# lim0606/pytorch-ardae-vae

Hardware: AMD Instinct MI355X
Metric: AR-DAE-VAE train-steps/sec (batch 512, nz_cdae 256) on dbMNIST (higher is better)
Workload: dtype f32; 1 GPU; BASELINE config #2: MNISTIPVAE mlp z=32 h=256 + cDAE mlp-grad h=256 L=3, global batch 512, nz_cdae 256 (131072 rows), dynamic binarisation on device, 1 cDAE + 1 VAE update per step; global_batch=512, nz_cdae=256, per_gpu_batch=512, parallelism=dp1

## Files before the change

pytorch-ardae-vae_amd/csrc/linear_narrow.hip:

```cpp
#include <stdlib.h>

#include "linear.h"
#include "profile.h"

namespace ardae {
namespace {

constexpr int NK = 32;

template <int EPI>
__global__ __launch_bounds__(256) void linear_narrow_kernel(const LinArgs a) {
  __shared__ float red[4];
  const int tid = threadIdx.x, lane = tid & 63, wave = tid >> 6;
  const int l31 = lane & 31, hh = lane >> 5;
  const int row0 = (blockIdx.x * 4 + wave) * 32;

  const float* xr = a.src[0].x + (size_t)(row0 + l31) * a.src[0].ld + 4 * hh;
  f32x4 av[NK];
#pragma unroll
  for (int c = 0; c < NK; ++c) av[c] = *reinterpret_cast<const f32x4*>(xr + 8 * c);

  const int col = min(l31, a.Nout - 1);
  const bool cok = l31 < a.Nout;
  const float bcol = a.bias ? a.bias[col] : 0.f;
  float sg[16], ev[16];
  if (EPI == EPI_DAE_LOSS) {
#pragma unroll
    for (int r = 0; r < 16; ++r) {
      const int row = row0 + (r & 3) + 8 * (r >> 2) + 4 * hh;
      sg[r] = a.sigma[row];
      ev[r] = a.eps[(size_t)row * a.ldeps + col];
    }
  }

  const float* bp = a.src[0].wp + lane * 4;
  f32x16 acc;
#pragma unroll
  for (int r = 0; r < 16; ++r) acc[r] = 0.f;
  f32x4 b0[8], b1[8];
#pragma unroll
  for (int u = 0; u < 8; ++u) b0[u] = *reinterpret_cast<const f32x4*>(bp + (size_t)u * 256);
#pragma unroll
  for (int g = 0; g < 4; g += 2) {
#pragma unroll
    for (int u = 0; u < 8; ++u) b1[u] = *reinterpret_cast<const f32x4*>(bp + (size_t)(8 * (g + 1) + u) * 256);
#pragma unroll
    for (int u = 0; u < 8; ++u)
#pragma unroll
      for (int q = 0; q < 4; ++q) acc = __builtin_amdgcn_mfma_f32_32x32x2f32(av[8 * g + u][q], b0[u][q], acc, 0, 0, 0);
    if (g + 2 < 4) {
#pragma unroll
      for (int u = 0; u < 8; ++u) b0[u] = *reinterpret_cast<const f32x4*>(bp + (size_t)(8 * (g + 2) + u) * 256);
    }
#pragma unroll
    for (int u = 0; u < 8; ++u)
#pragma unroll
      for (int q = 0; q < 4; ++q) acc = __builtin_amdgcn_mfma_f32_32x32x2f32(av[8 * (g + 1) + u][q], b1[u][q], acc, 0, 0, 0);
  }

  if (EPI == EPI_ACT) {
#pragma unroll
    for (int r = 0; r < 16; ++r) {
      const int row = row0 + (r & 3) + 8 * (r >> 2) + 4 * hh;
      if (cok) a.Y[(size_t)row * a.ldY + col] = acc[r] + bcol;
    }
  } else {
    float loss_part = 0.f;
#pragma unroll
    for (int r = 0; r < 16; ++r) {
      const int row = row0 + (r & 3) + 8 * (r >> 2) + 4 * hh;
      const float y = acc[r] + bcol;
      const float rho = sg[r] * y + ev[r];
      if (cok) {
        if (a.Y) a.Y[(size_t)row * a.ldY + col] = y;
        if (a.Y2) a.Y2[(size_t)row * a.ldY2 + col] = 2.f * sg[r] * rho * a.scale;
        loss_part += rho * rho;
      }
    }
#pragma unroll
    for (int off = 32; off > 0; off >>= 1) loss_part += __shfl_xor(loss_part, off);
    if (lane == 0) red[wave] = loss_part;
    __syncthreads();
    if (tid == 0) a.tile_loss[blockIdx.x] = (red[0] + red[1]) + (red[2] + red[3]);
  }
}

template <int EPI>
int launch_narrow(const LinArgs& a, hipStream_t st) {
  if (g_prof_enabled) {
    char name[64];
    snprintf(name, sizeof(name), "linear_narrow_kernel<%d>", EPI);
    const double tensors = EPI == EPI_DAE_LOSS ? (1.0 + (a.Y ? 1 : 0) + (a.Y2 ? 1 : 0)) : 1.0;
    prof_begin(st, name, 2.0 * a.M * (double)a.Nout * 256.0, 4.0 * ((double)a.M * 256.0 + tensors * a.M * (double)a.Nout + 256.0 * a.Nout));
  }
  hipLaunchKernelGGL((linear_narrow_kernel<EPI>), dim3(a.M / 128), dim3(256), 0, st, a);
  prof_end(st);
  ARDAE_LAUNCH_CHECK();
  return 0;
}

}

bool linear_narrow_eligible(const LinArgs& a, int epi) {
  static const bool on = !(debug_knob("ARDAE_NARROW") && atoi(debug_knob("ARDAE_NARROW")) == 0);
  if (!on || a.nsrc != 1 || a.src[0].K != 256 || a.Nout <= 0 || a.Nout > 32 || a.M <= 0 || (a.M % 128)) return false;
  if ((a.src[0].ld & 3) || (reinterpret_cast<uintptr_t>(a.src[0].x) & 15) || a.colsum != nullptr) return false;
  if (epi == EPI_ACT) return a.act == ACT_NONE && !a.rowbias && !a.rowscale && !a.Y2 && a.Y != nullptr;
  if (epi == EPI_DAE_LOSS) return a.tile_loss != nullptr && a.sigma != nullptr && a.eps != nullptr;
  return false;
}

int launch_linear_narrow(const LinArgs& a, int epi, hipStream_t st) {
  return epi == EPI_ACT ? launch_narrow<EPI_ACT>(a, st) : launch_narrow<EPI_DAE_LOSS>(a, st);
}

}
```

pytorch-ardae-vae_amd/csrc/wgrad_wide.hip:

```cpp
#include <stdlib.h>

#include "profile.h"
#include "wgrad.h"
#include "wgrad_wide_tiles.h"

namespace ardae {
namespace {

constexpr int WT = 256;
constexpr int WRC = 32;
constexpr int WCHUNK_BYTES = WRC * WT * 4;

template <int NA, int NB, int WOW>
struct WGeo {
  static constexpr int NA_ = NA, NB_ = NB;
  static constexpr int WIW = 4 / WOW;
  static constexpr int TO = NA * 32 * WOW, TI = NB * 32 * WIW;
  static constexpr int NM = NA * NB;
  static constexpr int XC4 = TI / 4;
  static constexpr int XRPP = 256 / XC4;
  static constexpr int NXP = WRC / XRPP;
  static constexpr int XCHUNK_BYTES = WRC * TI * 4;
  static constexpr int BUF_BYTES = WCHUNK_BYTES + XCHUNK_BYTES;
  static_assert(TO == WT, "the G staging layout assumes 256 output rows per tile");
};
using GeoSquare = WGeo<4, 4, 2>;
using GeoNarrow = WGeo<2, 1, 4>;

typedef __attribute__((address_space(3))) float lds_f32;



template <int OFF>
__device__ __forceinline__ void gload4(f32x4& dst, unsigned voff, const float* sbase) {
  asm volatile("s_nop 4\n\tglobal_load_dwordx4 %0, %1, %2 offset:%3" : "=v"(dst) : "v"(voff), "s"(sbase), "n"(OFF) : "memory");
}
template <int OFF>
__device__ __forceinline__ void gload1(float& dst, unsigned voff, const float* sbase) {
  asm volatile("s_nop 4\n\tglobal_load_dword %0, %1, %2 offset:%3" : "=v"(dst) : "v"(voff), "s"(sbase), "n"(OFF) : "memory");
}
template <int OFF>
__device__ __forceinline__ void lds_read1(float& dst, unsigned addr) {
  asm volatile("ds_read_b32 %0, %1 offset:%2" : "=v"(dst) : "v"(addr), "n"(OFF) : "memory");
}
template <int OFF>
__device__ __forceinline__ void lds_write4(unsigned addr, const f32x4& v) {
  asm volatile("ds_write_b128 %0, %1 offset:%2" ::"v"(addr), "v"(v), "n"(OFF) : "memory");
}

struct WwCtx {
  const float* gnext;
  const float* xnext;
  const float* rsnext;
  int ldg, ldx;
  unsigned gvoff, xvoff, rsvoff;
  unsigned gfrag, xfrag;
  unsigned gfrag_n, xfrag_n;
  unsigned gw, xw;
  float fb, fr;
};

template <class GEO>
struct Stage {
  static constexpr bool SQ = GEO::NM >= 8;
  static constexpr int PER = SQ ? 8 : 2;
  static constexpr int k_gl = 0, n_gl = 8 / PER;
  static constexpr int k_xl = k_gl + n_gl, n_xl = (GEO::NXP + PER - 1) / PER;
  static constexpr int k_rs = k_xl + n_xl, n_rs = 8 / PER;
  static constexpr int k_sum = 11;
  static constexpr int k_gw = 12, n_gw = SQ ? 1 : 2;
  static constexpr int k_xw = k_gw + n_gw;
  static_assert(k_rs + n_rs <= k_sum - 2 && k_xw <= 14, "stage schedule does not fit the chunk");
  static constexpr int count(int ks) {
    if (ks >= k_gl && ks < k_gl + n_gl) return PER;
    if (ks >= k_xl && ks < k_xl + n_xl) return (GEO::NXP - (ks - k_xl) * PER) < PER ? (GEO::NXP - (ks - k_xl) * PER) : PER;
    if (ks >= k_rs && ks < k_rs + n_rs) return PER;
    if (ks == k_sum) return 8;
    if (ks >= k_gw && ks < k_gw + n_gw) return 8 / n_gw;
    if (ks == k_xw) return GEO::NXP;
    return 0;
  }
};

template <class GEO, int KS, int J>
__device__ __forceinline__ void stage_op(f32x4 (&gv)[8], f32x4 (&xv)[GEO::NXP], float (&rs)[8], f32x4& bsum, f32x4& rsum, const WwCtx& c) {
  using ST = Stage<GEO>;
  if constexpr (KS >= ST::k_gl && KS < ST::k_gl + ST::n_gl) {
    constexpr int p = (KS - ST::k_gl) * ST::PER + J;
    gload4<0>(gv[p], c.gvoff, c.gnext + (size_t)(4 * p) * c.ldg);
  } else if constexpr (KS >= ST::k_xl && KS < ST::k_xl + ST::n_xl) {
    constexpr int p = (KS - ST::k_xl) * ST::PER + J;
    gload4<0>(xv[p], c.xvoff, c.xnext + (size_t)(GEO::XRPP * p) * c.ldx);
  } else if constexpr (KS >= ST::k_rs && KS < ST::k_rs + ST::n_rs) {
    constexpr int p = (KS - ST::k_rs) * ST::PER + J;
    gload1<16 * p>(rs[p], c.rsvoff, c.rsnext);
  } else if constexpr (KS == ST::k_sum) {
    if constexpr (J == 0) {
      asm volatile("s_waitcnt vmcnt(0)"
                   : "+v"(gv[0]), "+v"(gv[1]), "+v"(gv[2]), "+v"(gv[3]), "+v"(gv[4]), "+v"(gv[5]), "+v"(gv[6]), "+v"(gv[7])
                   :
                   : "memory");
      if constexpr (GEO::NXP == 8)
        asm volatile("s_waitcnt vmcnt(0)"
                     : "+v"(xv[0]), "+v"(xv[1]), "+v"(xv[2]), "+v"(xv[3]), "+v"(xv[4]), "+v"(xv[5]), "+v"(xv[6]), "+v"(xv[7])
                     :
                     : "memory");
      else asm volatile("s_waitcnt vmcnt(0)" : "+v"(xv[0]) : : "memory");
      asm volatile("s_waitcnt vmcnt(0)"
                   : "+v"(rs[0]), "+v"(rs[1]), "+v"(rs[2]), "+v"(rs[3]), "+v"(rs[4]), "+v"(rs[5]), "+v"(rs[6]), "+v"(rs[7])
                   :
                   : "memory");
    }
    bsum += gv[J] * c.fb;
    rsum += gv[J] * (rs[J] * c.fr);
  } else if constexpr (KS >= ST::k_gw && KS < ST::k_gw + ST::n_gw) {
    constexpr int p = (KS - ST::k_gw) * (8 / ST::n_gw) + J;
    lds_write4<p * 4096>(c.gw, gv[p]);
  } else if constexpr (KS == ST::k_xw) {
    lds_write4<J * GEO::XRPP * GEO::TI * 4>(c.xw, xv[J]);
  }
}

template <class GEO, int KS, int Q>
__device__ __forceinline__ void kstep_op(float (&A)[2][GEO::NA_], float (&B)[2][GEO::NB_], f32x4 (&gv)[8], f32x4 (&xv)[GEO::NXP], float (&rs)[8],
                                         f32x4& bsum, f32x4& rsum, const WwCtx& c) {
  constexpr int NA = GEO::NA_, NB = GEO::NB_;
  constexpr int nxt = (KS + 1) & 1;
  if constexpr (Q < NA) {
    if constexpr (KS < 15) lds_read1<(KS + 1) * 2048 + Q * 128>(A[nxt][Q], c.gfrag);
    else lds_read1<Q * 128>(A[nxt][Q], c.gfrag_n);
  } else if constexpr (Q < NA + NB) {
    constexpr int f = Q - NA;
    if constexpr (KS < 15) lds_read1<(KS + 1) * 2 * GEO::TI * 4 + f * 128>(B[nxt][f], c.xfrag);
    else lds_read1<f * 128>(B[nxt][f], c.xfrag_n);
  } else {
    stage_op<GEO, KS, Q - NA - NB>(gv, xv, rs, bsum, rsum, c);
  }
}

template <class GEO, int KS, int Q, int QEND>
__device__ __forceinline__ void kstep_ops(float (&A)[2][GEO::NA_], float (&B)[2][GEO::NB_], f32x4 (&gv)[8], f32x4 (&xv)[GEO::NXP], float (&rs)[8],
                                          f32x4& bsum, f32x4& rsum, const WwCtx& c) {
  if constexpr (Q < QEND) {
    kstep_op<GEO, KS, Q>(A, B, gv, xv, rs, bsum, rsum, c);
    kstep_ops<GEO, KS, Q + 1, QEND>(A, B, gv, xv, rs, bsum, rsum, c);
  }
}

template <class GEO, int KS, int S = 0>
__device__ __forceinline__ void kstep_mfmas(f32x16 (&acc)[GEO::NA_][GEO::NB_], float (&A)[2][GEO::NA_], float (&B)[2][GEO::NB_], f32x4 (&gv)[8],
                                            f32x4 (&xv)[GEO::NXP], float (&rs)[8], f32x4& bsum, f32x4& rsum, const WwCtx& c) {
  if constexpr (S < GEO::NM) {
    constexpr int a = S / GEO::NB_, b = S % GEO::NB_, cur = KS & 1;
    constexpr int total = GEO::NA_ + GEO::NB_ + Stage<GEO>::count(KS);
    constexpr int per = (total + GEO::NM - 1) / GEO::NM;
    constexpr int q0 = S * per < total ? S * per : total, q1 = (S + 1) * per < total ? (S + 1) * per : total;
    acc[a][b] = __builtin_amdgcn_mfma_f32_32x32x2f32(A[cur][a], B[cur][b], acc[a][b], 0, 0, 0);
    __builtin_amdgcn_sched_barrier(0);
    kstep_ops<GEO, KS, q0, q1>(A, B, gv, xv, rs, bsum, rsum, c);
    __builtin_amdgcn_sched_barrier(0);
    kstep_mfmas<GEO, KS, S + 1>(acc, A, B, gv, xv, rs, bsum, rsum, c);
  }
}

template <int N>
__device__ __forceinline__ void wait_frags(float (&v)[N]) {
  if constexpr (N == 4) asm volatile("s_waitcnt lgkmcnt(0)" : "+v"(v[0]), "+v"(v[1]), "+v"(v[2]), "+v"(v[3]) : : "memory");
  else if constexpr (N == 2) asm volatile("s_waitcnt lgkmcnt(0)" : "+v"(v[0]), "+v"(v[1]) : : "memory");
  else asm volatile("s_waitcnt lgkmcnt(0)" : "+v"(v[0]) : : "memory");
}

template <class GEO, int KS = 0>
__device__ __forceinline__ void chunk_ksteps(f32x16 (&acc)[GEO::NA_][GEO::NB_], float (&A)[2][GEO::NA_], float (&B)[2][GEO::NB_], f32x4 (&gv)[8],
                                             f32x4 (&xv)[GEO::NXP], float (&rs)[8], f32x4& bsum, f32x4& rsum, const WwCtx& c) {
  if constexpr (KS < 16) {
    constexpr int cur = KS & 1;
    wait_frags(A[cur]);
    wait_frags(B[cur]);
    if constexpr (KS == 15) __builtin_amdgcn_s_barrier();
    __builtin_amdgcn_sched_barrier(0);
    kstep_mfmas<GEO, KS>(acc, A, B, gv, xv, rs, bsum, rsum, c);
    chunk_ksteps<GEO, KS + 1>(acc, A, B, gv, xv, rs, bsum, rsum, c);
  }
}

template <class GEO>
__global__ __launch_bounds__(256, 1) void wgrad_wide_kernel(const WwBatchDev batch) {
  constexpr int NA = GEO::NA_, NB = GEO::NB_, NXP = GEO::NXP;
  __shared__ float lds[2 * GEO::BUF_BYTES / 4];
  const int tid = threadIdx.x, lane = tid & 63;
  const int wave = __builtin_amdgcn_readfirstlane(tid >> 6);
  const int l31 = lane & 31, hh = lane >> 5;
  const int wo = wave / GEO::WIW, wi = wave % GEO::WIW;
  const int ti = (int)blockIdx.x / batch.splits, split = (int)blockIdx.x - ti * batch.splits;
  const WwTile& T = batch.t[ti];

  const int cpp = T.M / WRC;
  const int ctot = cpp * T.npairs;
  const int cps = (ctot + batch.splits - 1) / batch.splits;
  const int c_begin = split * cps;
  const int c_end = c_begin + cps < ctot ? c_begin + cps : ctot;

  const unsigned lds0 = (unsigned)(uintptr_t)(lds_f32*)lds;
  const int sr = tid >> 6, sc4 = tid & 63;
  const int xr = tid / GEO::XC4, xc4 = tid % GEO::XC4;
  const unsigned gwbase = lds0 + (unsigned)((sr * WT + sc4 * 4) * 4);
  const unsigned xwbase = lds0 + WCHUNK_BYTES + (unsigned)((xr * GEO::TI + xc4 * 4) * 4);
  const unsigned gfrag0 = lds0 + (unsigned)((hh * WT + wo * NA * 32 + l31) * 4);
  const unsigned xfrag0 = lds0 + WCHUNK_BYTES + (unsigned)((hh * GEO::TI + wi * NB * 32 + l31) * 4);

  WwCtx c;
  auto chunk_ptrs = [&](int ch) {
    const int cc = ch < c_end ? ch : c_end - 1;
    const int pr = cc >= cpp ? 1 : 0;
    const int m0 = (cc - pr * cpp) * WRC;
    c.ldg = pr ? T.ldG[1] : T.ldG[0];
    c.ldx = pr ? T.ldX[1] : T.ldX[0];
    c.gnext = (pr ? T.G[1] : T.G[0]) + (size_t)m0 * c.ldg + T.o0;
    c.xnext = (pr ? T.X[1] : T.X[0]) + (size_t)m0 * c.ldx + T.i0;
    const bool vec = T.want_vec && pr == T.bias_pair && ch < c_end;
    c.fb = vec ? 1.f : 0.f;
    c.fr = (vec && T.rowscale) ? 1.f : 0.f;
    c.rsnext = T.rowscale ? T.rowscale + m0 : c.gnext;
    c.gvoff = (unsigned)((sr * c.ldg + sc4 * 4) * 4);
    c.xvoff = (unsigned)((xr * c.ldx + xc4 * 4) * 4);
    c.rsvoff = (unsigned)(sr * 4);
  };

  f32x16 acc[NA][NB];
#pragma unroll
  for (int a = 0; a < NA; ++a)
#pragma unroll
    for (int b = 0; b < NB; ++b)
#pragma unroll
      for (int r = 0; r < 16; ++r) acc[a][b][r] = 0.f;
  f32x4 bsum = {0.f, 0.f, 0.f, 0.f}, rsum = {0.f, 0.f, 0.f, 0.f};

  float A[2][NA], B[2][NB], rs[8];
  f32x4 gv[8], xv[NXP];
  if (c_begin < c_end) {
    chunk_ptrs(c_begin);
#pragma unroll
    for (int p = 0; p < 8; ++p) {
      gv[p] = *reinterpret_cast<const f32x4*>(c.gnext + (size_t)(4 * p + sr) * c.ldg + sc4 * 4);
      rs[p] = T.rowscale ? T.rowscale[(c.rsnext - T.rowscale) + 4 * p + sr] : 0.f;
    }
#pragma unroll
    for (int p = 0; p < NXP; ++p) xv[p] = *reinterpret_cast<const f32x4*>(c.xnext + (size_t)(GEO::XRPP * p + xr) * c.ldx + xc4 * 4);
#pragma unroll
    for (int p = 0; p < 8; ++p) {
      bsum += gv[p] * c.fb;
      rsum += gv[p] * (rs[p] * c.fr);
      *reinterpret_cast<f32x4*>(&lds[((4 * p + sr) * WT + sc4 * 4)]) = gv[p];
    }
#pragma unroll
    for (int p = 0; p < NXP; ++p) *reinterpret_cast<f32x4*>(&lds[WCHUNK_BYTES / 4 + (GEO::XRPP * p + xr) * GEO::TI + xc4 * 4]) = xv[p];
    __syncthreads();
#pragma unroll
    for (int f = 0; f < NA; ++f) A[0][f] = lds[hh * WT + wo * NA * 32 + f * 32 + l31];
#pragma unroll
    for (int f = 0; f < NB; ++f) B[0][f] = lds[WCHUNK_BYTES / 4 + hh * GEO::TI + wi * NB * 32 + f * 32 + l31];
    asm volatile("s_waitcnt vmcnt(0) lgkmcnt(0)" ::: "memory");

    int buf = 0;
    for (int ch = c_begin; ch < c_end; ++ch) {
      chunk_ptrs(ch + 1);
      const unsigned cur = (unsigned)buf * GEO::BUF_BYTES, oth = (unsigned)(buf ^ 1) * GEO::BUF_BYTES;
      c.gfrag = gfrag0 + cur; c.xfrag = xfrag0 + cur;
      c.gfrag_n = gfrag0 + oth; c.xfrag_n = xfrag0 + oth;
      c.gw = gwbase + oth; c.xw = xwbase + oth;
      chunk_ksteps<GEO, 0>(acc, A, B, gv, xv, rs, bsum, rsum, c);
      buf ^= 1;
    }
    wait_frags(A[0]);
    wait_frags(B[0]);
    asm volatile("s_waitcnt vmcnt(0) lgkmcnt(0)" ::: "memory");
  }

  float* __restrict__ part = T.partial + (size_t)split * T.O * T.I;
#pragma unroll
  for (int a = 0; a < NA; ++a) {
#pragma unroll
    for (int b = 0; b < NB; ++b) {
      const int i = T.i0 + wi * NB * 32 + b * 32 + l31;
#pragma unroll
      for (int r = 0; r < 16; ++r) {
        const int o = T.o0 + wo * NA * 32 + a * 32 + (r & 3) + 8 * (r >> 2) + 4 * hh;
        part[(size_t)o * T.I + i] = acc[a][b][r];
      }
    }
  }
  if (T.want_vec && T.i0 == 0) {
    __syncthreads();
    *reinterpret_cast<f32x4*>(&lds[sr * WT + sc4 * 4]) = bsum;
    *reinterpret_cast<f32x4*>(&lds[4 * WT + sr * WT + sc4 * 4]) = rsum;
    __syncthreads();
    const float s0 = (lds[tid] + lds[WT + tid]) + (lds[2 * WT + tid] + lds[3 * WT + tid]);
    const float s1 = (lds[4 * WT + tid] + lds[5 * WT + tid]) + (lds[6 * WT + tid] + lds[7 * WT + tid]);
    T.partial_vec[((size_t)split * 2 + 0) * T.O + T.o0 + tid] = s0;
    T.partial_vec[((size_t)split * 2 + 1) * T.O + T.o0 + tid] = s1;
  }
}

bool al16g(const void* p) { return (reinterpret_cast<uintptr_t>(p) & 15) == 0; }

}

int wgrad_wide_geometry(const WgradProblem& p) {
  static const bool off = debug_knob("ARDAE_WGRAD_WIDE") && atoi(debug_knob("ARDAE_WGRAD_WIDE")) == 0;
  if (off) return 0;
  if (p.O % WT || p.I % 32 || p.M % WRC || p.M < 64 * WRC) return 0;
  for (int k = 0; k < p.npairs; ++k) {
    if ((p.ldG[k] & 3) || (p.ldX[k] & 3) || !al16g(p.G[k]) || !al16g(p.X[k])) return 0;
    if ((int64_t)p.ldG[k] * 4 * 4 >= (int64_t)1 << 31 || (int64_t)p.ldX[k] * 32 * 4 >= (int64_t)1 << 31) return 0;
  }
  if (p.I % WT == 0) return 1;
  return p.I <= 64 ? 2 : 0;
}

bool wgrad_wide_eligible(const WgradProblem& p) { return wgrad_wide_geometry(p) != 0; }

template <class GEO>
int launch_wgrad_wide_geo(WgradProblem* probs, const int* idx, int n, hipStream_t st, const char* name) {
  if (n == 0) return 0;
  WwBatchDev b;
  memset(&b, 0, sizeof(b));
  int ntiles = 0, min_splits = 1 << 30;
  for (int k = 0; k < n; ++k) {
    const WgradProblem& p = probs[idx[k]];
    ntiles += (p.O / GEO::TO) * (p.I / GEO::TI);
    if (p.splits < min_splits) min_splits = p.splits;
  }
  ARDAE_CHECK_ARG(ntiles <= WW_MAX_TILES, "wgrad_wide: too many tiles (%d)", ntiles);
  int splits = 256 / ntiles;
  if (splits < 1) splits = 1;
  if (splits > min_splits) splits = min_splits;
  b.ntiles = ntiles;
  b.splits = splits;
  int t = 0;
  double fl = 0, by = 0;
  for (int k = 0; k < n; ++k) {
    WgradProblem& p = probs[idx[k]];
    p.splits = splits;
    for (int o0 = 0; o0 < p.O; o0 += GEO::TO)
      for (int i0 = 0; i0 < p.I; i0 += GEO::TI) {
        WwTile& w = b.t[t++];
        for (int q = 0; q < 2; ++q) {
          w.G[q] = p.G[q]; w.X[q] = p.X[q]; w.ldG[q] = p.ldG[q]; w.ldX[q] = p.ldX[q];
        }
        w.rowscale = p.rowscale; w.partial = p.partial; w.partial_vec = p.partial_vec;
        w.M = p.M; w.npairs = p.npairs; w.O = p.O; w.I = p.I; w.o0 = o0; w.i0 = i0;
        w.bias_pair = p.bias_pair; w.want_vec = (p.bias_pair >= 0 && p.partial_vec != nullptr) ? 1 : 0;
      }
    fl += 2.0 * p.npairs * (double)p.M * p.O * p.I;
    by += 4.0 * (p.npairs * (double)p.M * (p.O + p.I) + (double)splits * p.O * p.I);
  }
  bool x9 = GEO::TI == 256;
  for (int k = 0; x9 && k < n; ++k) x9 = wgrad_x9_eligible(probs[idx[k]]);
  if (g_prof_enabled) prof_begin(st, x9 ? "wgrad_x9_kernel<256x256>" : name, fl, by);
  if (x9) {
    ARDAE_TRY(launch_wgrad_x9(b, st));
  } else {
    hipLaunchKernelGGL(wgrad_wide_kernel<GEO>, dim3(ntiles * splits), dim3(256), 0, st, b);
  }
  prof_end(st);
  ARDAE_LAUNCH_CHECK();
  return n;
}

int launch_wgrad_wide(WgradProblem* probs, const int* idx, int n, hipStream_t st) {
  int sq[WGRAD_MAX_PROBLEMS], nr[WGRAD_MAX_PROBLEMS], nsq = 0, nnr = 0;
  for (int k = 0; k < n; ++k) {
    if (wgrad_wide_geometry(probs[idx[k]]) == 1) sq[nsq++] = idx[k];
    else nr[nnr++] = idx[k];
  }
  int rc = launch_wgrad_wide_geo<GeoSquare>(probs, sq, nsq, st, "wgrad_wide_kernel<256x256>");
  if (rc < 0) return rc;
  rc = launch_wgrad_wide_geo<GeoNarrow>(probs, nr, nnr, st, "wgrad_wide_kernel<256x32>");
  return rc < 0 ? rc : n;
}

}
```

Before: 223.8 train-steps/sec.

## Add persistent narrow-linear kernel and two-chunk-ahead prefetch in narrow wgrad

Adds a persistent version of the narrow (Nout<=32, K=256) linear kernel. It keeps the weight fragment in registers and double-buffers the next tile's activation rows while the current tile runs its MFMAs, which avoids reloading weights per tile and hides load latency. The narrow-geometry wgrad kernel now issues global loads two chunks ahead with two register sets and partial vmcnt waits, so fewer loads are exposed at each chunk boundary. The cost is higher register pressure, tricky waitcnt accounting and bias-vector bookkeeping, and a persistent grid hardcoded to 256 blocks.

```diff
diff --git a/pytorch-ardae-vae_amd/csrc/linear_narrow.hip b/pytorch-ardae-vae_amd/csrc/linear_narrow.hip
--- a/pytorch-ardae-vae_amd/csrc/linear_narrow.hip
+++ b/pytorch-ardae-vae_amd/csrc/linear_narrow.hip
@@ -85,6 +85,95 @@
   }
 }
 
+template <int EPI, int P>
+__device__ __forceinline__ void narrow_trip(const LinArgs& a, int t, int ntiles, f32x4 (&av)[2][NK], const f32x4 (&bw)[NK], float (&red)[2][4],
+                                            int tid, int lane, int wave, int col, bool cok, float bcol) {
+  const int l31 = lane & 31, hh = lane >> 5;
+  const int row0 = (t * 4 + wave) * 32;
+  float sg[16], ev[16];
+  if (EPI == EPI_DAE_LOSS) {
+#pragma unroll
+    for (int r = 0; r < 16; ++r) {
+      const int row = row0 + (r & 3) + 8 * (r >> 2) + 4 * hh;
+      sg[r] = a.sigma[row];
+      ev[r] = a.eps[(size_t)row * a.ldeps + col];
+    }
+  }
+  const int tn = t + (int)gridDim.x;
+  const float* xn = tn < ntiles ? a.src[0].x + (size_t)((tn * 4 + wave) * 32 + l31) * a.src[0].ld + 4 * hh : a.src[0].wp + 4 * hh;
+#pragma unroll
+  for (int c = 0; c < NK; ++c) av[P ^ 1][c] = *reinterpret_cast<const f32x4*>(xn + 8 * c);
+  __builtin_amdgcn_sched_barrier(0);
+
+  f32x16 acc;
+#pragma unroll
+  for (int r = 0; r < 16; ++r) acc[r] = 0.f;
+#pragma unroll
+  for (int c = 0; c < NK; ++c)
+#pragma unroll
+    for (int q = 0; q < 4; ++q) acc = __builtin_amdgcn_mfma_f32_32x32x2f32(av[P][c][q], bw[c][q], acc, 0, 0, 0);
+
+  if (EPI == EPI_ACT) {
+#pragma unroll
+    for (int r = 0; r < 16; ++r) {
+      const int row = row0 + (r & 3) + 8 * (r >> 2) + 4 * hh;
+      if (cok) a.Y[(size_t)row * a.ldY + col] = acc[r] + bcol;
+    }
+  } else {
+    float loss_part = 0.f;
+#pragma unroll
+    for (int r = 0; r < 16; ++r) {
+      const int row = row0 + (r & 3) + 8 * (r >> 2) + 4 * hh;
+      const float y = acc[r] + bcol;
+      const float rho = sg[r] * y + ev[r];
+      if (cok) {
+        if (a.Y) a.Y[(size_t)row * a.ldY + col] = y;
+        if (a.Y2) a.Y2[(size_t)row * a.ldY2 + col] = 2.f * sg[r] * rho * a.scale;
+        loss_part += rho * rho;
+      }
+    }
+#pragma unroll
+    for (int off = 32; off > 0; off >>= 1) loss_part += __shfl_xor(loss_part, off);
+    if (lane == 0) red[P][wave] = loss_part;
+    __syncthreads();
+    if (tid == 0) a.tile_loss[t] = (red[P][0] + red[P][1]) + (red[P][2] + red[P][3]);
+  }
+}
+
+template <int EPI>
+__global__ __launch_bounds__(256, 1) void linear_narrow_persistent_kernel(const LinArgs a, int ntiles) {
+  __shared__ float red[2][4];
+  const int tid = threadIdx.x, lane = tid & 63, wave = tid >> 6;
+  const int l31 = lane & 31, hh = lane >> 5;
+  int t = blockIdx.x;
+
+  f32x4 av[2][NK], bw[NK];
+  const float* xr = a.src[0].x + (size_t)((t * 4 + wave) * 32 + l31) * a.src[0].ld + 4 * hh;
+#pragma unroll
+  for (int c = 0; c < NK; ++c) av[0][c] = *reinterpret_cast<const f32x4*>(xr + 8 * c);
+  const float* bp = a.src[0].wp + lane * 4;
+#pragma unroll
+  for (int c = 0; c < NK; ++c) bw[c] = *reinterpret_cast<const f32x4*>(bp + (size_t)c * 256);
+  const int col = min(l31, a.Nout - 1);
+  const bool cok = l31 < a.Nout;
+  const float bcol = a.bias ? a.bias[col] : 0.f;
+
+  for (;;) {
+    narrow_trip<EPI, 0>(a, t, ntiles, av, bw, red, tid, lane, wave, col, cok, bcol);
+    t += (int)gridDim.x;
+    if (t >= ntiles) break;
+    narrow_trip<EPI, 1>(a, t, ntiles, av, bw, red, tid, lane, wave, col, cok, bcol);
+    t += (int)gridDim.x;
+    if (t >= ntiles) break;
+  }
+}
+
+constexpr int NARROW_CUS = 256;
+bool narrow_persistent(int ntiles) {
+  static const bool on = !(debug_knob("ARDAE_NARROW_PERSISTENT") && atoi(debug_knob("ARDAE_NARROW_PERSISTENT")) == 0);
+  return on && ntiles > 2 * NARROW_CUS;
+}
+
 template <int EPI>
 int launch_narrow(const LinArgs& a, hipStream_t st) {
   if (g_prof_enabled) {
@@ -93,7 +182,12 @@
     const double tensors = EPI == EPI_DAE_LOSS ? (1.0 + (a.Y ? 1 : 0) + (a.Y2 ? 1 : 0)) : 1.0;
     prof_begin(st, name, 2.0 * a.M * (double)a.Nout * 256.0, 4.0 * ((double)a.M * 256.0 + tensors * a.M * (double)a.Nout + 256.0 * a.Nout));
   }
-  hipLaunchKernelGGL((linear_narrow_kernel<EPI>), dim3(a.M / 128), dim3(256), 0, st, a);
+  const int ntiles = a.M / 128;
+  if (narrow_persistent(ntiles)) {
+    hipLaunchKernelGGL((linear_narrow_persistent_kernel<EPI>), dim3(NARROW_CUS), dim3(256), 0, st, a, ntiles);
+  } else {
+    hipLaunchKernelGGL((linear_narrow_kernel<EPI>), dim3(ntiles), dim3(256), 0, st, a);
+  }
   prof_end(st);
   ARDAE_LAUNCH_CHECK();
   return 0;
diff --git a/pytorch-ardae-vae_amd/csrc/wgrad_wide.hip b/pytorch-ardae-vae_amd/csrc/wgrad_wide.hip
--- a/pytorch-ardae-vae_amd/csrc/wgrad_wide.hip
+++ b/pytorch-ardae-vae_amd/csrc/wgrad_wide.hip
@@ -82,33 +82,42 @@
   }
 };
 
-template <class GEO, int KS, int J>
-__device__ __forceinline__ void stage_op(f32x4 (&gv)[8], f32x4 (&xv)[GEO::NXP], float (&rs)[8], f32x4& bsum, f32x4& rsum, const WwCtx& c) {
+template <class GEO, int AH, int LS, int KS, int J>
+__device__ __forceinline__ void stage_op(f32x4 (&gva)[AH][8], f32x4 (&xva)[AH][GEO::NXP], float (&rsa)[AH][8], f32x4& bsum, f32x4& rsum,
+                                         const WwCtx& c) {
   using ST = Stage<GEO>;
+  constexpr bool SAME = AH == 1 || LS == 2;
+  constexpr int L = LS & 1, CS = SAME ? L : L ^ 1, NEWER = SAME ? 0 : 8 + GEO::NXP + 8;
+  f32x4 (&gl)[8] = gva[L];
+  f32x4 (&xl)[GEO::NXP] = xva[L];
+  float (&rl)[8] = rsa[L];
+  f32x4 (&gv)[8] = gva[CS];
+  f32x4 (&xv)[GEO::NXP] = xva[CS];
+  float (&rs)[8] = rsa[CS];
   if constexpr (KS >= ST::k_gl && KS < ST::k_gl + ST::n_gl) {
     constexpr int p = (KS - ST::k_gl) * ST::PER + J;
-    gload4<0>(gv[p], c.gvoff, c.gnext + (size_t)(4 * p) * c.ldg);
+    gload4<0>(gl[p], c.gvoff, c.gnext + (size_t)(4 * p) * c.ldg);
   } else if constexpr (KS >= ST::k_xl && KS < ST::k_xl + ST::n_xl) {
     constexpr int p = (KS - ST::k_xl) * ST::PER + J;
-    gload4<0>(xv[p], c.xvoff, c.xnext + (size_t)(GEO::XRPP * p) * c.ldx);
+    gload4<0>(xl[p], c.xvoff, c.xnext + (size_t)(GEO::XRPP * p) * c.ldx);
   } else if constexpr (KS >= ST::k_rs && KS < ST::k_rs + ST::n_rs) {
     constexpr int p = (KS - ST::k_rs) * ST::PER + J;
-    gload1<16 * p>(rs[p], c.rsvoff, c.rsnext);
+    gload1<16 * p>(rl[p], c.rsvoff, c.rsnext);
   } else if constexpr (KS == ST::k_sum) {
     if constexpr (J == 0) {
-      asm volatile("s_waitcnt vmcnt(0)"
+      asm volatile("s_waitcnt vmcnt(%[n])"
                    : "+v"(gv[0]), "+v"(gv[1]), "+v"(gv[2]), "+v"(gv[3]), "+v"(gv[4]), "+v"(gv[5]), "+v"(gv[6]), "+v"(gv[7])
-                   :
+                   : [n] "n"(NEWER)
                    : "memory");
       if constexpr (GEO::NXP == 8)
-        asm volatile("s_waitcnt vmcnt(0)"
+        asm volatile("s_waitcnt vmcnt(%[n])"
                      : "+v"(xv[0]), "+v"(xv[1]), "+v"(xv[2]), "+v"(xv[3]), "+v"(xv[4]), "+v"(xv[5]), "+v"(xv[6]), "+v"(xv[7])
-                     :
+                     : [n] "n"(NEWER)
                      : "memory");
-      else asm volatile("s_waitcnt vmcnt(0)" : "+v"(xv[0]) : : "memory");
-      asm volatile("s_waitcnt vmcnt(0)"
+      else asm volatile("s_waitcnt vmcnt(%[n])" : "+v"(xv[0]) : [n] "n"(NEWER) : "memory");
+      asm volatile("s_waitcnt vmcnt(%[n])"
                    : "+v"(rs[0]), "+v"(rs[1]), "+v"(rs[2]), "+v"(rs[3]), "+v"(rs[4]), "+v"(rs[5]), "+v"(rs[6]), "+v"(rs[7])
-                   :
+                   : [n] "n"(NEWER)
                    : "memory");
     }
     bsum += gv[J] * c.fb;
@@ -121,9 +130,9 @@
   }
 }
 
-template <class GEO, int KS, int Q>
-__device__ __forceinline__ void kstep_op(float (&A)[2][GEO::NA_], float (&B)[2][GEO::NB_], f32x4 (&gv)[8], f32x4 (&xv)[GEO::NXP], float (&rs)[8],
-                                         f32x4& bsum, f32x4& rsum, const WwCtx& c) {
+template <class GEO, int AH, int LS, int KS, int Q>
+__device__ __forceinline__ void kstep_op(float (&A)[2][GEO::NA_], float (&B)[2][GEO::NB_], f32x4 (&gv)[AH][8], f32x4 (&xv)[AH][GEO::NXP],
+                                         float (&rs)[AH][8], f32x4& bsum, f32x4& rsum, const WwCtx& c) {
   constexpr int NA = GEO::NA_, NB = GEO::NB_;
   constexpr int nxt = (KS + 1) & 1;
   if constexpr (Q < NA) {
@@ -134,22 +143,22 @@
     if constexpr (KS < 15) lds_read1<(KS + 1) * 2 * GEO::TI * 4 + f * 128>(B[nxt][f], c.xfrag);
     else lds_read1<f * 128>(B[nxt][f], c.xfrag_n);
   } else {
-    stage_op<GEO, KS, Q - NA - NB>(gv, xv, rs, bsum, rsum, c);
-  }
-}
-
-template <class GEO, int KS, int Q, int QEND>
-__device__ __forceinline__ void kstep_ops(float (&A)[2][GEO::NA_], float (&B)[2][GEO::NB_], f32x4 (&gv)[8], f32x4 (&xv)[GEO::NXP], float (&rs)[8],
-                                          f32x4& bsum, f32x4& rsum, const WwCtx& c) {
+    stage_op<GEO, AH, LS, KS, Q - NA - NB>(gv, xv, rs, bsum, rsum, c);
+  }
+}
+
+template <class GEO, int AH, int LS, int KS, int Q, int QEND>
+__device__ __forceinline__ void kstep_ops(float (&A)[2][GEO::NA_], float (&B)[2][GEO::NB_], f32x4 (&gv)[AH][8], f32x4 (&xv)[AH][GEO::NXP],
+                                          float (&rs)[AH][8], f32x4& bsum, f32x4& rsum, const WwCtx& c) {
   if constexpr (Q < QEND) {
-    kstep_op<GEO, KS, Q>(A, B, gv, xv, rs, bsum, rsum, c);
-    kstep_ops<GEO, KS, Q + 1, QEND>(A, B, gv, xv, rs, bsum, rsum, c);
-  }
-}
-
-template <class GEO, int KS, int S = 0>
-__device__ __forceinline__ void kstep_mfmas(f32x16 (&acc)[GEO::NA_][GEO::NB_], float (&A)[2][GEO::NA_], float (&B)[2][GEO::NB_], f32x4 (&gv)[8],
-                                            f32x4 (&xv)[GEO::NXP], float (&rs)[8], f32x4& bsum, f32x4& rsum, const WwCtx& c) {
+    kstep_op<GEO, AH, LS, KS, Q>(A, B, gv, xv, rs, bsum, rsum, c);
+    kstep_ops<GEO, AH, LS, KS, Q + 1, QEND>(A, B, gv, xv, rs, bsum, rsum, c);
+  }
+}
+
+template <class GEO, int AH, int LS, int KS, int S = 0>
+__device__ __forceinline__ void kstep_mfmas(f32x16 (&acc)[GEO::NA_][GEO::NB_], float (&A)[2][GEO::NA_], float (&B)[2][GEO::NB_], f32x4 (&gv)[AH][8],
+                                            f32x4 (&xv)[AH][GEO::NXP], float (&rs)[AH][8], f32x4& bsum, f32x4& rsum, const WwCtx& c) {
   if constexpr (S < GEO::NM) {
     constexpr int a = S / GEO::NB_, b = S % GEO::NB_, cur = KS & 1;
     constexpr int total = GEO::NA_ + GEO::NB_ + Stage<GEO>::count(KS);
@@ -157,9 +166,19 @@
     constexpr int q0 = S * per < total ? S * per : total, q1 = (S + 1) * per < total ? (S + 1) * per : total;
     acc[a][b] = __builtin_amdgcn_mfma_f32_32x32x2f32(A[cur][a], B[cur][b], acc[a][b], 0, 0, 0);
     __builtin_amdgcn_sched_barrier(0);
-    kstep_ops<GEO, KS, q0, q1>(A, B, gv, xv, rs, bsum, rsum, c);
+    kstep_ops<GEO, AH, LS, KS, q0, q1>(A, B, gv, xv, rs, bsum, rsum, c);
     __builtin_amdgcn_sched_barrier(0);
-    kstep_mfmas<GEO, KS, S + 1>(acc, A, B, gv, xv, rs, bsum, rsum, c);
+    kstep_mfmas<GEO, AH, LS, KS, S + 1>(acc, A, B, gv, xv, rs, bsum, rsum, c);
+  }
+}
+
+template <class GEO, int P = 0>
+__device__ __forceinline__ void issue_chunk_loads(f32x4 (&gv)[8], f32x4 (&xv)[GEO::NXP], float (&rs)[8], const WwCtx& c) {
+  if constexpr (P < 8) {
+    gload4<0>(gv[P], c.gvoff, c.gnext + (size_t)(4 * P) * c.ldg);
+    if constexpr (P < GEO::NXP) gload4<0>(xv[P], c.xvoff, c.xnext + (size_t)(GEO::XRPP * P) * c.ldx);
+    gload1<16 * P>(rs[P], c.rsvoff, c.rsnext);
+    issue_chunk_loads<GEO, P + 1>(gv, xv, rs, c);
   }
 }
 
@@ -170,21 +189,21 @@
   else asm volatile("s_waitcnt lgkmcnt(0)" : "+v"(v[0]) : : "memory");
 }
 
-template <class GEO, int KS = 0>
-__device__ __forceinline__ void chunk_ksteps(f32x16 (&acc)[GEO::NA_][GEO::NB_], float (&A)[2][GEO::NA_], float (&B)[2][GEO::NB_], f32x4 (&gv)[8],
-                                             f32x4 (&xv)[GEO::NXP], float (&rs)[8], f32x4& bsum, f32x4& rsum, const WwCtx& c) {
+template <class GEO, int AH, int LS, int KS = 0>
+__device__ __forceinline__ void chunk_ksteps(f32x16 (&acc)[GEO::NA_][GEO::NB_], float (&A)[2][GEO::NA_], float (&B)[2][GEO::NB_], f32x4 (&gv)[AH][8],
+                                             f32x4 (&xv)[AH][GEO::NXP], float (&rs)[AH][8], f32x4& bsum, f32x4& rsum, const WwCtx& c) {
   if constexpr (KS < 16) {
     constexpr int cur = KS & 1;
     wait_frags(A[cur]);
     wait_frags(B[cur]);
     if constexpr (KS == 15) __builtin_amdgcn_s_barrier();
     __builtin_amdgcn_sched_barrier(0);
-    kstep_mfmas<GEO, KS>(acc, A, B, gv, xv, rs, bsum, rsum, c);
-    chunk_ksteps<GEO, KS + 1>(acc, A, B, gv, xv, rs, bsum, rsum, c);
-  }
-}
-
-template <class GEO>
+    kstep_mfmas<GEO, AH, LS, KS>(acc, A, B, gv, xv, rs, bsum, rsum, c);
+    chunk_ksteps<GEO, AH, LS, KS + 1>(acc, A, B, gv, xv, rs, bsum, rsum, c);
+  }
+}
+
+template <class GEO, int AH>
 __global__ __launch_bounds__(256, 1) void wgrad_wide_kernel(const WwBatchDev batch) {
   constexpr int NA = GEO::NA_, NB = GEO::NB_, NXP = GEO::NXP;
   __shared__ float lds[2 * GEO::BUF_BYTES / 4];
@@ -210,7 +229,7 @@
   const unsigned xfrag0 = lds0 + WCHUNK_BYTES + (unsigned)((hh * GEO::TI + wi * NB * 32 + l31) * 4);
 
   WwCtx c;
-  auto chunk_ptrs = [&](int ch) {
+  auto chunk_ptrs = [&](int ch, int use) {
     const int cc = ch < c_end ? ch : c_end - 1;
     const int pr = cc >= cpp ? 1 : 0;
     const int m0 = (cc - pr * cpp) * WRC;
@@ -218,7 +237,7 @@
     c.ldx = pr ? T.ldX[1] : T.ldX[0];
     c.gnext = (pr ? T.G[1] : T.G[0]) + (size_t)m0 * c.ldg + T.o0;
     c.xnext = (pr ? T.X[1] : T.X[0]) + (size_t)m0 * c.ldx + T.i0;
-    const bool vec = T.want_vec && pr == T.bias_pair && ch < c_end;
+    const bool vec = T.want_vec && (use >= cpp ? 1 : 0) == T.bias_pair && use < c_end;
     c.fb = vec ? 1.f : 0.f;
     c.fr = (vec && T.rowscale) ? 1.f : 0.f;
     c.rsnext = T.rowscale ? T.rowscale + m0 : c.gnext;
@@ -236,10 +255,13 @@
       for (int r = 0; r < 16; ++r) acc[a][b][r] = 0.f;
   f32x4 bsum = {0.f, 0.f, 0.f, 0.f}, rsum = {0.f, 0.f, 0.f, 0.f};
 
-  float A[2][NA], B[2][NB], rs[8];
-  f32x4 gv[8], xv[NXP];
+  float A[2][NA], B[2][NB], rsa[AH][8];
+  f32x4 gva[AH][8], xva[AH][NXP];
   if (c_begin < c_end) {
-    chunk_ptrs(c_begin);
+    f32x4 (&gv)[8] = gva[0];
+    f32x4 (&xv)[NXP] = xva[0];
+    float (&rs)[8] = rsa[0];
+    chunk_ptrs(c_begin, c_begin);
 #pragma unroll
     for (int p = 0; p < 8; ++p) {
       gv[p] = *reinterpret_cast<const f32x4*>(c.gnext + (size_t)(4 * p + sr) * c.ldg + sc4 * 4);
@@ -263,18 +285,44 @@
     asm volatile("s_waitcnt vmcnt(0) lgkmcnt(0)" ::: "memory");
 
     int buf = 0;
-    for (int ch = c_begin; ch < c_end; ++ch) {
-      chunk_ptrs(ch + 1);
+    auto lds_ptrs = [&]() {
       const unsigned cur = (unsigned)buf * GEO::BUF_BYTES, oth = (unsigned)(buf ^ 1) * GEO::BUF_BYTES;
       c.gfrag = gfrag0 + cur; c.xfrag = xfrag0 + cur;
       c.gfrag_n = gfrag0 + oth; c.xfrag_n = xfrag0 + oth;
       c.gw = gwbase + oth; c.xw = xwbase + oth;
-      chunk_ksteps<GEO, 0>(acc, A, B, gv, xv, rs, bsum, rsum, c);
       buf ^= 1;
+    };
+    if constexpr (AH == 1) {
+      for (int ch = c_begin; ch < c_end; ++ch) {
+        chunk_ptrs(ch + 1, ch + 1);
+        lds_ptrs();
+        chunk_ksteps<GEO, 1, 0>(acc, A, B, gva, xva, rsa, bsum, rsum, c);
+      }
+    } else {
+      int ch = c_begin;
+      if ((c_end - c_begin) & 1) {
+        chunk_ptrs(ch + 1, ch + 1);
+        lds_ptrs();
+        chunk_ksteps<GEO, 2, 2>(acc, A, B, gva, xva, rsa, bsum, rsum, c);
+        ++ch;
+      }
+      if (ch < c_end) {
+        chunk_ptrs(ch + 1, ch + 1);
+        issue_chunk_loads<GEO>(gva[0], xva[0], rsa[0], c);
+        for (; ch < c_end; ch += 2) {
+          chunk_ptrs(ch + 2, ch + 1);
+          lds_ptrs();
+          chunk_ksteps<GEO, 2, 1>(acc, A, B, gva, xva, rsa, bsum, rsum, c);
+          chunk_ptrs(ch + 3, ch + 2);
+          lds_ptrs();
+          chunk_ksteps<GEO, 2, 0>(acc, A, B, gva, xva, rsa, bsum, rsum, c);
+        }
+      }
     }
     wait_frags(A[0]);
     wait_frags(B[0]);
     asm volatile("s_waitcnt vmcnt(0) lgkmcnt(0)" ::: "memory");
+    __builtin_amdgcn_sched_barrier(0);
   }
 
   float* __restrict__ part = T.partial + (size_t)split * T.O * T.I;
@@ -361,7 +409,14 @@
   if (x9) {
     ARDAE_TRY(launch_wgrad_x9(b, st));
   } else {
-    hipLaunchKernelGGL(wgrad_wide_kernel<GEO>, dim3(ntiles * splits), dim3(256), 0, st, b);
+    static const bool ahead1 = debug_knob("ARDAE_WGRAD_AHEAD") && atoi(debug_knob("ARDAE_WGRAD_AHEAD")) == 1;
+    if constexpr (GEO::TI == 256) {
+      hipLaunchKernelGGL((wgrad_wide_kernel<GEO, 1>), dim3(ntiles * splits), dim3(256), 0, st, b);
+    } else if (ahead1) {
+      hipLaunchKernelGGL((wgrad_wide_kernel<GEO, 1>), dim3(ntiles * splits), dim3(256), 0, st, b);
+    } else {
+      hipLaunchKernelGGL((wgrad_wide_kernel<GEO, 2>), dim3(ntiles * splits), dim3(256), 0, st, b);
+    }
   }
   prof_end(st);
   ARDAE_LAUNCH_CHECK();
```

After: 224.5 train-steps/sec, median of 6. Within noise of the previous version (+0.3%).
